# at-aaims/OmniFed

Hardware: AMD Instinct MI355X
Metric: GB/s device-resident QSGD encode+decode, Llama-400M grads, 1/2/4/8 GPUs (higher is better)
Workload: dtype f32; 1 GPU; llama400m QSGD encode+decode, bit_width 4 (16 levels, int8 wire), philox draws, client weighting fused (alpha = batch_samples = rank + 1), one client per GPU; tensors=183, elements_per_client=401122304, bit_width=4, parallelism=clients1

## Files before the change

omnifed_amd/csrc/omf_qsgd_bracket.hip:

```cpp
#include <algorithm>
#include <cstdlib>

#include "omf_bracket.h"
#include "omf_common.h"
#include "omf_plan.h"
#include "omf_qsgd_dec.h"
#include "omf_qsgd_dev.h"
#include "omf_qsgd_enc.h"

using namespace omf;
using namespace omf::plan_layout;

namespace {

constexpr int kSpecV = 4;
static_assert(kSpecBlk == (int64_t)kSpecV * kThreads * 4, "4096 elements per block");
constexpr int kSpecPerWaveWide = 32;
__host__ __device__ constexpr int spec_slot_words(int pw) { return pw == kSpecPerWave ? kSpecSlot : kWaves * pw; }
constexpr int64_t kSpecExact = 16384;

struct SpecArgs {
  EncArgs e;
  const int64_t* begins;
  const int64_t* sizes;
  const SpecBrItem* br_items;
  const SpecFoldItem* fold_items;
  SpecBracket* br;
  uint64_t* seg_part;
  uint32_t* fold_cnt;
  uint64_t* partials;
  uint32_t* heads;
  uint32_t* slots;
  float4* recs;
  uint32_t* flags;
  uint32_t* status;
  uint64_t* ngran;
  uint64_t wait_ticks;
  uint32_t dbg;
  float divisor;
  float zsig;
  float* xout;
  uint32_t epoch;
  uint32_t wide;
  double* br_part;
  uint64_t* brgran;
  uint32_t* br_cnt;
  int64_t nblocks;
  const void* aq;
  const float* anorm;
  float* aout;
  float alevels, ainv;
  int32_t awidth;
};

template <int AW, bool FULL>
__device__ __forceinline__ int4 acc_load(const void* q, int64_t e, int64_t end) {
  if (AW == 1) {
    const int8_t* q8 = static_cast<const int8_t*>(q);
    if (FULL || e + 4 <= end)
      return make_int4(__builtin_nontemporal_load(reinterpret_cast<const int32_t*>(q8 + e)), 0, 0, 0);
    uint32_t w = 0;
    for (int c = 0; c < 3; ++c)
      if (e + c < end) w |= (uint32_t)(uint8_t)q8[e + c] << (8 * c);
    return make_int4((int32_t)w, 0, 0, 0);
  }
  const int32_t* q32 = static_cast<const int32_t*>(q);
  if (FULL || e + 4 <= end) {
    const i32x4_t t = __builtin_nontemporal_load(reinterpret_cast<const i32x4_t*>(q32 + e));
    return make_int4(t[0], t[1], t[2], t[3]);
  }
  int4 r = make_int4(0, 0, 0, 0);
  if (e < end) r.x = q32[e];
  if (e + 1 < end) r.y = q32[e + 1];
  if (e + 2 < end) r.z = q32[e + 2];
  return r;
}

template <int AW>
__device__ __forceinline__ float4 acc_add4(float4 v, int4 raw, float norm, float alevels, float ainv) {
  int32_t qi[4];
  if (AW == 1) {
    qsgd_split_i8(raw.x, qi);
  } else {
    qi[0] = raw.x; qi[1] = raw.y; qi[2] = raw.z; qi[3] = raw.w;
  }
  float y[4];
#pragma unroll
  for (int c = 0; c < 4; ++c)
    y[c] = ainv != 0.0f ? qsgd_dec_elem<true>(norm, qi[c], alevels, ainv) : qsgd_dec_elem<false>(norm, qi[c], alevels, ainv);
  return make_float4(__fadd_rn(v.x, y[0]), __fadd_rn(v.y, y[1]), __fadd_rn(v.z, y[2]), __fadd_rn(v.w, y[3]));
}

__device__ __forceinline__ float4 br_value(const SpecArgs& a, float4 v, int64_t e, int64_t end, int32_t t) {
  if (!a.aq) return v;
  const float nrm = a.anorm[t];
  if (a.awidth == 32) return acc_add4<4>(v, acc_load<4, false>(a.aq, e, end), nrm, a.alevels, a.ainv);
  return acc_add4<1>(v, acc_load<1, false>(a.aq, e, end), nrm, a.alevels, a.ainv);
}

__device__ __forceinline__ uint32_t spec_hash(uint32_t a, uint32_t b) {
  uint32_t h = a * 0x9E3779B1u ^ (b + 0x7F4A7C15u) * 0x85EBCA77u;
  h ^= h >> 15; h *= 0x2C1B3C6Du; h ^= h >> 12; h *= 0x297A2D39u; h ^= h >> 15;
  return h;
}


__device__ __forceinline__ float4 scale_alpha(float4 v, float alpha) {
  if (alpha != 1.0f) {
    v.x = __fmul_rn(v.x, alpha); v.y = __fmul_rn(v.y, alpha);
    v.z = __fmul_rn(v.z, alpha); v.w = __fmul_rn(v.w, alpha);
  }
  return v;
}

__device__ __forceinline__ float4 spec_prologue(float4 v, float alpha, float divisor, uint32_t fmt) {
  v = scale_alpha(v, alpha);
  if (fmt && alpha != 1.0f) v = round_fmt4(v, fmt);
  if (divisor != 0.0f) {
    v.x = __fdiv_rn(v.x, divisor); v.y = __fdiv_rn(v.y, divisor);
    v.z = __fdiv_rn(v.z, divisor); v.w = __fdiv_rn(v.w, divisor);
  }
  return v;
}



template <int N>
__device__ __forceinline__ bool arrive_last(uint64_t* all, int32_t row, int64_t slot, const double (&v)[N],
                                            uint32_t* cnt, int32_t t, int parts) {
  uint64_t* mine = all + N * ((int64_t)row * parts + slot);
#pragma unroll
  for (int i = 0; i < N; ++i) st_agent(mine + i, (uint64_t)__double_as_longlong(v[i]));
  drain_vmem();
  const bool last = add_agent(&cnt[t], 1u) == (uint32_t)(parts - 1);
  if (last) __hip_atomic_store(&cnt[t], 0u, __ATOMIC_RELAXED, __HIP_MEMORY_SCOPE_AGENT);
  return last;
}
template <int N>
__device__ __forceinline__ bool arrive_last_block(uint64_t* all, int32_t row, int64_t slot, const double (&v)[N],
                                                  uint32_t* cnt, int32_t t, int parts, uint32_t& s_last) {
  if (threadIdx.x == 0) s_last = arrive_last(all, row, slot, v, cnt, t, parts) ? 1u : 0u;
  __syncthreads();
  return s_last != 0u;
}
__device__ __forceinline__ void combine_parts(const uint64_t* all, int32_t row, int parts, double (&S)[2]) {
  S[0] = S[1] = 0.0;
  for (int g = 0; g < parts; ++g) {
    const uint64_t* bp = all + 2 * ((int64_t)row * parts + g);
    S[0] += __longlong_as_double((long long)ld_agent(bp));
    S[1] += __longlong_as_double((long long)ld_agent(bp + 1));
  }
}

constexpr int kBrThreads = 1024;
constexpr int kBrWaves = kBrThreads / 64;

__device__ __forceinline__ double br_sum(double v, double* lds) {
  v = wave_sum_f64(v);
  if ((threadIdx.x & 63) == 0) lds[threadIdx.x >> 6] = v;
  __syncthreads();
  double s = 0.0;
#pragma unroll
  for (int w = 0; w < kBrWaves; ++w) s += lds[w];
  __syncthreads();
  return s;
}

template <int RUN, bool AQ, int NT = kBrThreads, int PASSES = 8>
__device__ __forceinline__ void bracket_sample(const SpecArgs& a, const float* __restrict__ x, int32_t t, int64_t tb,
                                               int64_t n, int64_t R, int part, int parts, double& s1, double& s2) {
  constexpr int LPR = RUN / 4, RPP = NT / LPR, PER_ROUND = RPP * PASSES;
  const int64_t base = n / R, rem = n % R;
  const int j = threadIdx.x & (LPR - 1);
  const float alpha = a.e.alpha;
  for (int64_t rb = (int64_t)part * PER_ROUND; rb < R; rb += (int64_t)parts * PER_ROUND) {
    float4 v[PASSES];
    bool live[PASSES];
    auto run_pos = [&](int i) {
      const int64_t r0 = rb + (int64_t)i * RPP + (threadIdx.x / LPR);
      const int64_t r = r0 < R ? r0 : 0;
      const int64_t lo = r * base + min(r, rem), len = base + (r < rem ? 1 : 0);
      return ((lo + (int64_t)(spec_hash((uint32_t)r, (uint32_t)t) % (uint32_t)(len - (RUN - 1)))) & ~(int64_t)3) + 4 * j;
    };
#pragma unroll
    for (int i = 0; i < PASSES; ++i) {
      live[i] = rb + (int64_t)i * RPP + (threadIdx.x / LPR) < R;
      v[i] = *reinterpret_cast<const float4*>(x + run_pos(i));
    }
    if (AQ) {
#pragma unroll
      for (int i = 0; i < PASSES; ++i) v[i] = br_value(a, v[i], tb + run_pos(i), tb + n, t);
    }
#pragma unroll
    for (int i = 0; i < PASSES; ++i) {
      float sr = live[i] ? sq4(spec_prologue(v[i], alpha, a.divisor, a.e.fmt), 0.0f) : 0.0f;
#pragma unroll
      for (int o = LPR / 2; o > 0; o >>= 1) sr += __shfl_xor(sr, o, LPR);
      if (live[i] && j == 0) {
        s1 += (double)sr;
        s2 += (double)sr * (double)sr;
      }
    }
  }
}

__device__ SpecBracket bracket_from_sums(const SpecArgs& a, bool exact, int64_t n, int64_t R, int run, double S1,
                                         double S2);

template <bool WIDE, bool AQ>
__device__ __forceinline__ void spec_bracket_body(const SpecArgs& a, const SpecBrItem* __restrict__ items,
                                                  double* red, uint32_t& s_last) {
  const int parts = WIDE ? kBrParts : 1;
  const int part = (int)(blockIdx.x % (unsigned)parts);
  const SpecBrItem bi = items[blockIdx.x / (unsigned)parts];
  const int32_t t = bi.tensor;
  const int64_t tb = bi.begin, n = bi.n;
  const float* __restrict__ x = a.e.x + tb;
  const float alpha = a.e.alpha;
  double s1 = 0.0, s2 = 0.0;
  const bool exact = n <= kSpecExact;
  const int64_t R = WIDE ? (int64_t)bi.Rw : (int64_t)bi.R;
  if (exact) {
    constexpr int PER = (int)(kSpecExact / (4 * kBrThreads));
    float4 v[PER];
    const int64_t nq = n & ~(int64_t)3;
#pragma unroll
    for (int i = 0; i < PER; ++i) {
      const int64_t e = 4 * ((int64_t)i * kBrThreads + threadIdx.x);
      v[i] = nq ? *reinterpret_cast<const float4*>(x + (e < nq ? e : 0)) : make_float4(0.f, 0.f, 0.f, 0.f);
    }
#pragma unroll
    for (int i = 0; i < PER; ++i) {
      const int64_t e = 4 * ((int64_t)i * kBrThreads + threadIdx.x);
      if (e >= nq) {
        v[i] = make_float4(0.f, 0.f, 0.f, 0.f);
        if (e < n) {
          v[i].x = x[e];
          if (e + 1 < n) v[i].y = x[e + 1];
          if (e + 2 < n) v[i].z = x[e + 2];
        }
      }
    }
    if (AQ) {
#pragma unroll
      for (int i = 0; i < PER; ++i) {
        const int64_t e = 4 * ((int64_t)i * kBrThreads + threadIdx.x);
        if (e < n) v[i] = br_value(a, v[i], tb + e, tb + n, t);
      }
    }
    float acc = 0.0f;
#pragma unroll
    for (int i = 0; i < PER; ++i) acc = sq4(spec_prologue(v[i], alpha, a.divisor, a.e.fmt), acc);
    s1 = acc;
  } else {
    bracket_sample<WIDE ? kSpecRunWide : kSpecRun, AQ>(a, x, t, tb, n, R, part, parts, s1, s2);
  }
  if (exact && part != 0) return;
  double S[2];
  S[0] = br_sum(s1, red);
  S[1] = br_sum(s2, red);
  if (!exact && parts > 1) {
    uint64_t* bp = reinterpret_cast<uint64_t*>(a.br_part);
    if (!arrive_last_block(bp, t, part, S, a.br_cnt, t, parts, s_last) || threadIdx.x != 0) return;
    combine_parts(bp, t, parts, S);
  }
  if (threadIdx.x != 0) return;
  a.br[t] = bracket_from_sums(a, exact, n, R, WIDE ? kSpecRunWide : kSpecRun, S[0], S[1]);
}

__device__ SpecBracket bracket_from_sums(const SpecArgs& a, bool exact, int64_t n, int64_t R, int run, double S1,
                                         double S2) {
  double ss, k;
  if (exact) {
    ss = S1;
    k = 0x1p-12;
  } else {
    const double Rd = (double)R, m = S1 / Rd;
    const double var = fmax(0.0, (S2 - Rd * m * m) / (Rd - 1.0));
    ss = S1 * ((double)n / ((double)run * Rd));
    k = (double)a.zsig * sqrt(var / Rd) / m + 0x1p-10;
  }
  const uint32_t fmt = a.e.fmt;
  const double kf = fmt == kFmtBF16 ? 0x1p-7 + 0x1p-14 : (fmt == kFmtF16 ? 0x1p-10 + 0x1p-20 : 0.0);
  const double mf = fmt == kFmtBF16 ? 0x1p-8 + 0x1p-16 : (fmt == kFmtF16 ? 0x1p-11 + 0x1p-22 : 0.0);
  k += kf;
  SpecBracket o{0.f, 0.f, 0.f, 0.f, 1u, {0u, 0u, 0u}};
  if (ss > 0.0 && ss < 1e300 && k < 0.5) {
    const float n_lo = nextafterf((float)sqrt(ss * (1.0 - k)), 0.0f);
    const float n_hi = nextafterf((float)sqrt(ss * (1.0 + k)), INFINITY);
    if (n_lo >= 0x1p-90f && n_hi < INFINITY) {
      const double L = (double)a.e.levels;
      o.n_lo = n_lo;
      o.n_hi = n_hi;
      o.c_lo = nextafterf((float)(L / (double)n_hi * (1.0 - 0x1p-20) * (1.0 - mf)), 0.0f);
      o.c_hi = nextafterf((float)(L / (double)n_lo * (1.0 + 0x1p-20) * (1.0 + mf)), INFINITY);
      o.mode = 0u;
    }
  }
  return o;
}

template <bool WIDE, bool AQ>
__global__ __launch_bounds__(kBrThreads) void qsgd_spec_bracket(SpecArgs a, const SpecBrItem* __restrict__ items) {
  __shared__ double red[kBrWaves];
  __shared__ uint32_t s_last;
  spec_bracket_body<WIDE, AQ>(a, items, red, s_last);
}
__global__ __launch_bounds__(kBrThreads) __attribute__((amdgpu_waves_per_eu(8))) void qsgd_spec_bracket_wide(
    SpecArgs a, const SpecBrItem* __restrict__ items) {
  __shared__ double red[kBrWaves];
  __shared__ uint32_t s_last;
  spec_bracket_body<true, false>(a, items, red, s_last);
}

__device__ __forceinline__ float raise_u(float u) {
  return __uint_as_float(max(__float_as_uint(u), 0x32800000u));
}
__device__ __forceinline__ void spec_quad(float4 x, float4 u, float c_lo, float c_hi, int32_t (&q)[4], uint64_t& und) {
  const float xs[4] = {x.x, x.y, x.z, x.w}, us[4] = {u.x, u.y, u.z, u.w};
#pragma unroll
  for (int c = 0; c < 4; ++c) {
    const float ax = fabsf(xs[c]);
    const float kl = ceilf(fmaf(ax, c_lo, -raise_u(us[c])));
    const float kh = ceilf(fmaf(ax, c_hi, -us[c]));
    und |= __builtin_amdgcn_fcmpf(kl, kh, 14 );
    q[c] = (int32_t)copysignf(kh, xs[c]);
  }
}

__device__ __forceinline__ void spec_quad_fmt(float4 x, float4 u, float c_lo, float c_hi, float dl, int32_t (&q)[4],
                                              uint64_t& und) {
  const float xs[4] = {x.x, x.y, x.z, x.w}, us[4] = {u.x, u.y, u.z, u.w};
#pragma unroll
  for (int c = 0; c < 4; ++c) {
    const float ax = fabsf(xs[c]);
    const float kl = ceilf(fmaf(ax, c_lo, -(raise_u(us[c]) + dl)));
    const float kh = ceilf(fmaf(ax, c_hi, dl - us[c]));
    und |= __builtin_amdgcn_fcmpf(kl, kh, 14 );
    q[c] = (int32_t)copysignf(kh, xs[c]);
  }
}


template <int WIDTH, bool FULL, bool DIV, uint32_t FMT, int AW = 0, int PW = kSpecPerWave, class GetBr>
__device__ __forceinline__ void spec_block(const SpecArgs& a, int64_t blk, int64_t b, int64_t end, int32_t t,
                                           int64_t tb, GetBr get_br, uint32_t* slot, uint64_t* part, float anorm,
                                           int tid) {
  const EncArgs& e = a.e;
  const int lane = tid & 63;
  const int wave = __builtin_amdgcn_readfirstlane(tid >> 6);
  float4 v[kSpecV];
  load_f4<kSpecV, FULL, true>(e.x, b, end, v, tid);
  int4 araw[AW ? kSpecV : 1];
  if (AW) {
#pragma unroll
    for (int k = 0; k < kSpecV; ++k)
      araw[k] = acc_load<AW ? AW : 1, FULL>(a.aq, b + 4 * ((int64_t)k * kThreads + tid), end);
  }
  float4 uu[4];
  philox_rows(e, b, tb, t, 0, uu, tid);
  const float alpha = e.alpha;
  float acc = 0.0f;
#pragma unroll
  for (int k = 0; k < kSpecV; ++k) {
    v[k] = mul4(v[k], alpha);
    if (FMT != kFmtF32 && alpha != 1.0f) v[k] = round_fmt4(v[k], FMT);
    if (AW) {
      v[k] = acc_add4<AW ? AW : 1>(v[k], araw[k], anorm, a.alevels, a.ainv);
      if (a.aout) {
        const int64_t el = b + 4 * ((int64_t)k * kThreads + tid);
        if (FULL || el + 4 <= end) {
          store_nt(a.aout + el, v[k]);
        } else if (el < end) {
          a.aout[el] = v[k].x;
          if (el + 1 < end) a.aout[el + 1] = v[k].y;
          if (el + 2 < end) a.aout[el + 2] = v[k].z;
        }
      }
    }
    if (DIV) {
      const float d = a.divisor;
      v[k].x = __fdiv_rn(v[k].x, d); v[k].y = __fdiv_rn(v[k].y, d);
      v[k].z = __fdiv_rn(v[k].z, d); v[k].w = __fdiv_rn(v[k].w, d);
      const int64_t el = b + 4 * ((int64_t)k * kThreads + tid);
      if (FULL || el + 4 <= end) {
        store_nt(a.xout + el, v[k]);
      } else if (el < end) {
        a.xout[el] = v[k].x;
        if (el + 1 < end) a.xout[el + 1] = v[k].y;
        if (el + 2 < end) a.xout[el + 2] = v[k].z;
      }
    }
    acc = sq4(v[k], acc);
  }
  const SpecBracket br = get_br();
  uint32_t cnt = 0;
  {
    uint32_t* list = slot + PW * wave;
#pragma unroll
    for (int k = 0; k < kSpecV; ++k) {
      const int64_t el = b + 4 * ((int64_t)k * kThreads + tid);
      const bool live = FULL || el < end;
      int32_t qq[4];
      uint64_t m = 0;
      if (FMT == kFmtF32) spec_quad(v[k], uu[k], br.c_lo, br.c_hi, qq, m);
      else spec_quad_fmt(v[k], uu[k], br.c_lo, br.c_hi, FMT == kFmtF16 ? 0x1p-25f * e.levels : 0.0f, qq, m);
      if (live) store_quad<WIDTH, FULL>(e, el, end, qq);
      if (!FULL) m &= __builtin_amdgcn_ballot_w64(live);
      if (m) {
        const bool und = (m >> lane) & 1ull;
        const uint32_t pos =
            cnt + __builtin_amdgcn_mbcnt_hi((uint32_t)(m >> 32), __builtin_amdgcn_mbcnt_lo((uint32_t)m, 0u));
        if (live && und && pos < (uint32_t)PW) {
          list[pos] = (uint32_t)(el >> 2);
          float4* rec = a.recs + 2 * ((blk * kWaves + wave) * PW + pos);
          rec[0] = v[k];
          rec[1] = uu[k];
        }
        cnt += (uint32_t)__popcll(m);
      }
    }
  }
  const double s = wave_sum_f64((double)acc);
  if (lane == 0) {
    *part = (uint64_t)__double_as_longlong(s);
    a.heads[blk * kWaves + wave] = ((uint32_t)t << 8) | min(cnt, (uint32_t)PW);
    if (cnt > (uint32_t)PW)
      __hip_atomic_fetch_or(&a.flags[t], 1u, __ATOMIC_RELAXED, __HIP_MEMORY_SCOPE_AGENT);
  }
}

template <int WIDTH, bool DIV, uint32_t FMT = kFmtF32, int AW = 0, int PW = kSpecPerWave, int WPB = kWaves>
__global__ __launch_bounds__(64 * WPB) void qsgd_spec_quant(SpecArgs a, const SpecBracket* __restrict__ brs,
                                                            const int64_t* __restrict__ begins,
                                                            const float* __restrict__ anorms) {
  static_assert(kWaves % WPB == 0, "a block's waves split evenly");
  constexpr int kPer = kWaves / WPB;
  const int64_t blk = blockIdx.x / kPer;
  const int tid = (int)(blockIdx.x % kPer) * 64 * WPB + (int)threadIdx.x;
  const Item it = a.e.items[blk >> 2];
  const SpecBracket br = brs[it.tensor];
  const int64_t tb = begins[it.tensor];
  const float anorm = AW ? anorms[it.tensor] : 0.0f;
  const int64_t b = it.begin + (blk & 3) * kSpecBlk;
  const int wave = tid >> 6;
  uint32_t* slot = a.slots + blk * spec_slot_words(PW);
  uint64_t* part = a.partials + blk * kWaves + wave;
  if (b >= it.end) {
    if ((tid & 63) == 0) {
      *part = 0ull;
      a.heads[blk * kWaves + wave] = (uint32_t)it.tensor << 8;
    }
    return;
  }
  const int64_t end = min(b + kSpecBlk, it.end);
  auto get_br = [&]() { return br; };
  if (end - b == kSpecBlk)
    spec_block<WIDTH, true, DIV, FMT, AW, PW>(a, blk, b, end, it.tensor, tb, get_br, slot, part, anorm, tid);
  else
    spec_block<WIDTH, false, DIV, FMT, AW, PW>(a, blk, b, end, it.tensor, tb, get_br, slot, part, anorm, tid);
}

#ifndef OMF_WFB_PASSES
#define OMF_WFB_PASSES 8
#endif
constexpr int kPassesW = OMF_WFB_PASSES;

template <int NT>
__device__ __forceinline__ double whole_sumsq(const SpecArgs& a, const float* __restrict__ x, int64_t n) {
  double s = 0.0;
  for (int64_t r0 = 0; r0 < n; r0 += 16 * NT) {
    float4 v[4];
#pragma unroll
      for (int i = 0; i < 4; ++i) {
        const int64_t e = r0 + 4 * ((int64_t)i * NT + threadIdx.x);
        v[i] = e + 4 <= n ? *reinterpret_cast<const float4*>(x + e) : make_float4(0.f, 0.f, 0.f, 0.f);
        if (e < n && e + 4 > n) {
          v[i].x = x[e];
          if (e + 1 < n) v[i].y = x[e + 1];
          if (e + 2 < n) v[i].z = x[e + 2];
        }
      }
    float acc = 0.0f;
#pragma unroll
    for (int i = 0; i < 4; ++i) acc = sq4(spec_prologue(v[i], a.e.alpha, a.divisor, a.e.fmt), acc);
    s += (double)acc;
  }
  return s;
}

template <int NT, int PARTS, int RUN, int PASSES>
__device__ __forceinline__ void spec_bracket_part(const SpecArgs& a, const SpecBrItem* __restrict__ items, int64_t wg) {
  static_assert(NT == 64 || NT == kThreads, "one wave, or block_sum_f64's workgroup");
  const int part = (int)(wg % PARTS);
  const SpecBrItem bi = items[wg / PARTS];
  const int32_t t = bi.tensor;
  const int64_t tb = bi.begin, n = bi.n, R = RUN == kSpecRunWide ? bi.Rw : bi.R;
  const float* __restrict__ x = a.e.x + tb;
  const bool exact = n <= kSpecExact;
  if (exact && part != 0) return;
  double s1 = 0.0, s2 = 0.0;
  if (exact) s1 = whole_sumsq<NT>(a, x, n);
  else bracket_sample<RUN, false, NT, PASSES>(a, x, t, tb, n, R, part, PARTS, s1, s2);
  double S[2];
  if constexpr (NT == 64) {
    S[0] = wave_sum_f64(s1);
    S[1] = wave_sum_f64(s2);
    if (threadIdx.x != 0) return;
  } else {
    __shared__ double red[kWaves];
    S[0] = block_sum_f64(s1, red);
    S[1] = block_sum_f64(s2, red);
  }
  if (!exact) {
    uint64_t* bp = reinterpret_cast<uint64_t*>(a.br_part);
    bool last;
    if constexpr (NT == 64) {
      last = arrive_last(bp, t, part, S, a.br_cnt, t, PARTS);
    } else {
      __shared__ uint32_t s_last;
      last = arrive_last_block(bp, t, part, S, a.br_cnt, t, PARTS, s_last);
    }
    if (!last) return;
    combine_parts(bp, t, PARTS, S);
  }
  if (threadIdx.x != 0) return;
  const SpecBracket o = bracket_from_sums(a, exact, n, R, RUN, S[0], S[1]);
  a.br[t] = o;
  const uint64_t ep = (uint64_t)a.epoch << 32;
  st_agent(&a.brgran[2 * t], ep | __float_as_uint(o.c_lo));
  st_agent(&a.brgran[2 * t + 1], ep | __float_as_uint(o.c_hi));
}

__device__ __forceinline__ SpecBracket fb_poll(const SpecArgs& a, int32_t t) {
  uint64_t g0 = ld_agent(&a.brgran[2 * t]), g1 = ld_agent(&a.brgran[2 * t + 1]);
  if ((uint32_t)(g0 >> 32) != a.epoch || (uint32_t)(g1 >> 32) != a.epoch) {
    const uint64_t t0 = wall_clock64(), min_polls = a.wait_ticks >> 10;
    uint64_t polls = 0;
    for (int k = 0;; k = min(k + 1, 6)) {
      if (k < 2) __builtin_amdgcn_s_sleep(2);
      else __builtin_amdgcn_s_sleep(8);
      g0 = ld_agent(&a.brgran[2 * t]);
      g1 = ld_agent(&a.brgran[2 * t + 1]);
      if ((uint32_t)(g0 >> 32) == a.epoch && (uint32_t)(g1 >> 32) == a.epoch) break;
      if (++polls > min_polls && wall_clock64() - t0 > a.wait_ticks) {
        __hip_atomic_fetch_or(&a.flags[t], 2u, __ATOMIC_RELAXED, __HIP_MEMORY_SCOPE_AGENT);
        g0 = g1 = 0;
        break;
      }
    }
  }
  return SpecBracket{__uint_as_float((uint32_t)g0), __uint_as_float((uint32_t)g1), 0.f, 0.f, 0u, {0u, 0u, 0u}};
}

template <int WIDTH, bool DIV, int PW>
__device__ __forceinline__ void fused_pass_block(const SpecArgs& a, int64_t blk, int tid,
                                                 const int64_t* __restrict__ begins) {
  const Item it = a.e.items[blk >> 2];
  const int32_t t = it.tensor;
  const int64_t tb = begins[t];
  const int64_t b = it.begin + (blk & 3) * kSpecBlk;
  const int wave = tid >> 6;
  uint32_t* slot = a.slots + blk * spec_slot_words(PW);
  uint64_t* part = a.partials + blk * kWaves + wave;
  if (b >= it.end) {
    if ((tid & 63) == 0) {
      *part = 0ull;
      a.heads[blk * kWaves + wave] = (uint32_t)t << 8;
    }
    return;
  }
  auto get_br = [&]() { return fb_poll(a, t); };
  const int64_t end = min(b + kSpecBlk, it.end);
  if (end - b == kSpecBlk)
    spec_block<WIDTH, true, DIV, kFmtF32, 0, PW>(a, blk, b, end, t, tb, get_br, slot, part, 0.0f, tid);
  else
    spec_block<WIDTH, false, DIV, kFmtF32, 0, PW>(a, blk, b, end, t, tb, get_br, slot, part, 0.0f, tid);
}

template <int WIDTH, bool DIV>
__global__ __launch_bounds__(kThreads) void qsgd_spec_quant_fb(SpecArgs a, const SpecBrItem* __restrict__ bitems,
                                                               int64_t nbrw, const int64_t* __restrict__ begins) {
  if ((int64_t)blockIdx.x < nbrw) {
    spec_bracket_part<kThreads, kFbParts, kSpecRun, 4>(a, bitems, blockIdx.x);
    return;
  }
  fused_pass_block<WIDTH, DIV, kSpecPerWave>(a, (int64_t)blockIdx.x - nbrw, (int)threadIdx.x, begins);
}

template <int WIDTH, bool DIV>
__global__ __launch_bounds__(64) void qsgd_spec_quant_wfb(SpecArgs a, const SpecBrItem* __restrict__ bitems,
                                                          int64_t nbrw, const int64_t* __restrict__ begins) {
  if ((int64_t)blockIdx.x < nbrw) {
    spec_bracket_part<64, kWfbParts, kSpecRunWide, kPassesW>(a, bitems, blockIdx.x);
    return;
  }
  const int64_t wgi = (int64_t)blockIdx.x - nbrw;
  fused_pass_block<WIDTH, DIV, kSpecPerWaveWide>(a, wgi / kWaves, (int)(wgi % kWaves) * 64 + (int)threadIdx.x, begins);
}

__device__ void spec_fold(const SpecArgs& a, const SpecFoldItem& fi) {
  __shared__ double red[kWaves];
  __shared__ uint32_t s_last;
  const int32_t t = fi.tensor;
  constexpr int U = kSpecSeg / kThreads;
  double v[U];
#pragma unroll
  for (int i = 0; i < U; ++i) {
    const int64_t j = fi.p_begin + threadIdx.x + (int64_t)i * kThreads;
    const double d = __longlong_as_double((long long)a.partials[j < fi.p_end ? j : fi.p_begin]);
    v[i] = j < fi.p_end ? d : 0.0;
  }
  double p = 0.0;
#pragma unroll
  for (int i = 0; i < U; ++i) p += v[i];
  double tot = block_sum_f64(p, red);
  if (fi.nsegs > 1) {
    const double seg[1] = {tot};
    if (!arrive_last_block(a.seg_part, 0, fi.sbase + fi.seg, seg, a.fold_cnt, t, fi.nsegs, s_last)) return;
    double q = 0.0;
    for (int j = threadIdx.x; j < fi.nsegs; j += kThreads)
      q += __longlong_as_double((long long)ld_agent(&a.seg_part[fi.sbase + j]));
    tot = block_sum_f64(q, red);
  }
  if (threadIdx.x != 0) return;
  const float norm = finish_norm(tot, a.e.fmt);
  a.e.norm_out[t] = norm;
  const SpecBracket br = a.br[t];
  const uint32_t fl = a.flags[t];
  const bool ok = br.mode == 0u && fl == 0u && norm >= br.n_lo && norm <= br.n_hi;
  a.status[t] = ok ? 0u : 1u;
  if (fl) a.flags[t] = 0u;
  st_agent(&a.ngran[t], ((uint64_t)((a.epoch << 1) | (ok ? 0u : 1u)) << 32) | __float_as_uint(norm));
}

__device__ __forceinline__ bool spec_norm_wait(const SpecArgs& a, int32_t t, float& norm, bool& bad) {
  uint64_t g = ld_agent(&a.ngran[t]);
  if ((uint32_t)(g >> 33) != a.epoch) {
    const uint64_t t0 = wall_clock64();
    const uint64_t min_polls = a.wait_ticks >> 10;
    uint64_t polls = 0;
    for (int k = 0;; k = min(k + 1, 6)) {
      if (k < 2) __builtin_amdgcn_s_sleep(4);
      else if (k < 4) __builtin_amdgcn_s_sleep(16);
      else __builtin_amdgcn_s_sleep(64);
      g = ld_agent(&a.ngran[t]);
      if ((uint32_t)(g >> 33) == a.epoch) break;
      if (++polls > min_polls && wall_clock64() - t0 > a.wait_ticks) {
        __hip_atomic_fetch_or(a.e.err, 4u, __ATOMIC_RELAXED, __HIP_MEMORY_SCOPE_AGENT);
        return false;
      }
    }
  }
  norm = __uint_as_float((uint32_t)g);
  bad = ((g >> 32) & 1u) != 0u;
  return true;
}

template <int WIDTH, int PW = kSpecPerWave, int FT = 1>
__global__ __launch_bounds__(kThreads) void qsgd_spec_finish(SpecArgs a, const SpecFoldItem* __restrict__ fold_items,
                                                             int32_t nfold, const Item* __restrict__ items,
                                                             const int64_t* __restrict__ begins,
                                                             const uint32_t* __restrict__ slots,
                                                             const float4* __restrict__ recs,
                                                             const uint32_t* __restrict__ heads) {
  if ((int32_t)blockIdx.x < nfold) {
    if (!(a.dbg & 16u)) spec_fold(a, fold_items[blockIdx.x]);
    return;
  }
  constexpr int BPW = kThreads / (kWaves * FT);
  __shared__ uint32_t s_rep[BPW];
  __shared__ float s_rep_norm[BPW];
  __shared__ uint32_t s_nrep;
  const EncArgs& e = a.e;
  const int64_t fb = (int64_t)blockIdx.x - nfold;
  if (threadIdx.x == 0) s_nrep = 0u;
  const int64_t ws = (fb * kThreads + threadIdx.x) / FT;
  const uint32_t sub = (uint32_t)(threadIdx.x % FT);
  const int64_t blk = ws / kWaves;
  const int w = (int)(ws % kWaves);
  bool rep = false;
  float rep_norm = 0.0f;
  if (blk < a.nblocks) {
    const uint32_t head = heads[ws];
    const uint32_t cnt = head & 0xffu;
    const int32_t t = (int32_t)(head >> 8);
    const bool leader = w == 0 && sub == 0;
    if ((cnt > 0u || leader) && !(a.dbg & 8u)) {
      constexpr int PRE = FT > 1 ? PW / FT : 0;
      uint32_t qv[PRE > 0 ? PRE : 1];
      float4 rx[PRE > 0 ? PRE : 1], ru[PRE > 0 ? PRE : 1];
      const uint32_t jl = cnt > 0u ? cnt - 1u : 0u;
#pragma unroll
      for (int k = 0; k < PRE; ++k) {
        const uint32_t j = min(sub + (uint32_t)(k * FT), jl);
        qv[k] = slots[blk * spec_slot_words(PW) + PW * w + j];
        rx[k] = recs[2 * (ws * PW + j)];
        ru[k] = recs[2 * (ws * PW + j) + 1];
      }
      const Item it = items[blk >> 2];
      float norm;
      bool bad;
      if (spec_norm_wait(a, t, norm, bad)) {
        const int64_t b = it.begin + (blk & 3) * kSpecBlk, end = min(b + kSpecBlk, it.end);
        const Divisor dv(norm, e.fmt);
#pragma unroll
        for (int k = 0; k < PRE; ++k) {
          if (sub + (uint32_t)(k * FT) >= cnt) break;
          int32_t qq[4];
          qsgd_quad<false>(rx[k], ru[k], dv, e.levels, false, qq);
          if (!(a.dbg & 4u)) store_quad<WIDTH>(e, 4 * (int64_t)qv[k], end, qq);
        }
        for (uint32_t j = sub + (uint32_t)(PRE * FT); j < cnt; j += FT) {
          const uint32_t q = slots[blk * spec_slot_words(PW) + PW * w + j];
          const float4* rec = recs + 2 * (ws * PW + j);
          int32_t qq[4];
          qsgd_quad<false>(rec[0], rec[1], dv, e.levels, false, qq);
          if (!(a.dbg & 4u)) store_quad<WIDTH>(e, 4 * (int64_t)q, end, qq);
        }
        rep = leader && bad;
        rep_norm = norm;
      }
    }
  }
  __syncthreads();
  if (rep) {
    const uint32_t i = atomicAdd(&s_nrep, 1u);
    s_rep[i] = (uint32_t)(blk - fb * BPW);
    s_rep_norm[i] = rep_norm;
  }
  if (!__syncthreads_or(rep)) return;
  const uint32_t nrep = s_nrep;
  EncArgs er = e;
  if (a.divisor != 0.0f) {
    er.x = a.xout;
    er.alpha = 1.0f;
  }
  for (uint32_t r = 0; r < nrep; ++r) {
    const int64_t rb = fb * BPW + s_rep[r];
    const Item it = items[rb >> 2];
    const int64_t b = it.begin + (rb & 3) * kSpecBlk;
    if (b < it.end)
      quant_sub<WIDTH, false, kSpecV>(er, b, min(b + kSpecBlk, it.end), begins[it.tensor], it.tensor, s_rep_norm[r]);
  }
}

}

static int ensure_wide(omf_plan* p, hipStream_t st) {
  if (p->d_spec_slots_w) return OMF_OK;
  const size_t nt = (size_t)p->nt, nb = (size_t)p->n_spec_blocks;
  Carve c;
  c.raw(p->d_spec_slots_w, (size_t)spec_slot_words(kSpecPerWaveWide) * nb);
  c.raw(p->d_spec_recs_w, 2 * (size_t)kWaves * kSpecPerWaveWide * nb);
  c.raw(p->d_spec_br_part, 2 * (size_t)kBrParts * nt);
  c.zero(p->d_spec_br_cnt, nt);
  return make_buffers(p, c, st);
}

static int ensure_fused_bracket(omf_plan* p, hipStream_t st) {
  if (p->d_spec_fb_part) return OMF_OK;
  const size_t nt = (size_t)p->nt;
  Carve c;
  c.raw(p->d_spec_fb_part, 2 * (size_t)std::max(kFbParts, kWfbParts) * nt);
  c.zero(p->d_spec_fb_cnt, nt);
  c.zero(p->d_spec_brgran, 2 * nt);
  return make_buffers(p, c, st);
}

int omf::bracket::launch(omf_plan* p, const EncCall& c, const Choice& ch) {
  using BracketKernel = void (*)(SpecArgs, const SpecBrItem*);
  using PassKernel = void (*)(SpecArgs, const SpecBracket*, const int64_t*, const float*);
  using FusedKernel = void (*)(SpecArgs, const SpecBrItem*, int64_t, const int64_t*);
  using FinishKernel = void (*)(SpecArgs, const SpecFoldItem*, int32_t, const Item*, const int64_t*, const uint32_t*,
                                const float4*, const uint32_t*);
  constexpr int PWW = kSpecPerWaveWide;
#ifndef OMF_FIX_FT
#define OMF_FIX_FT 4
#endif
  constexpr int FT = OMF_FIX_FT;
  static const BracketKernel k_bracket[2] = {qsgd_spec_bracket<false, false>, qsgd_spec_bracket<false, true>};
  static const FusedKernel k_fb[2] = {qsgd_spec_quant_fb<1, false>, qsgd_spec_quant_fb<1, true>};
  static const FusedKernel k_wfb[2][2] = {{qsgd_spec_quant_wfb<1, false>, qsgd_spec_quant_wfb<1, true>},
                                          {qsgd_spec_quant_wfb<4, false>, qsgd_spec_quant_wfb<4, true>}};
  static const PassKernel k_pass[2][2] = {{qsgd_spec_quant<1, false>, qsgd_spec_quant<1, true>},
                                          {qsgd_spec_quant<4, false>, qsgd_spec_quant<4, true>}};
  static const PassKernel k_pass_half[2] = {qsgd_spec_quant<1, false, kFmtBF16>, qsgd_spec_quant<1, false, kFmtF16>};
  static const PassKernel k_pass_last[2] = {qsgd_spec_quant<1, true, kFmtF32, 1>,
                                            qsgd_spec_quant<1, true, kFmtF32, 4>};
  static const PassKernel k_pass_wide[2][2][2] = {
      {{qsgd_spec_quant<1, false, kFmtF32, 0, PWW, 1>, qsgd_spec_quant<1, true, kFmtF32, 0, PWW, 1>},
       {qsgd_spec_quant<4, false, kFmtF32, 0, PWW, 1>, qsgd_spec_quant<4, true, kFmtF32, 0, PWW, 1>}},
      {{qsgd_spec_quant<1, false, kFmtF32, 0, PWW>, qsgd_spec_quant<1, true, kFmtF32, 0, PWW>},
       {qsgd_spec_quant<4, false, kFmtF32, 0, PWW>, qsgd_spec_quant<4, true, kFmtF32, 0, PWW>}}};
  static const FinishKernel k_finish[2][2] = {{qsgd_spec_finish<1>, qsgd_spec_finish<4>},
                                              {qsgd_spec_finish<1, PWW, FT>, qsgd_spec_finish<4, PWW, FT>}};
  static const size_t plds_w = [] { const char* v = omf::knob("OMF_SPEC_LDS_W"); return v ? (size_t)atoi(v) : (size_t)10240; }();
  static const size_t plds_n = [] { const char* v = omf::knob("OMF_SPEC_LDS"); return v ? (size_t)atoi(v) : (size_t)24576; }();
  static const bool wpb4 = [] { const char* v = omf::knob("OMF_SPEC_WPB"); return v && atoi(v) == 4; }();

  const hipStream_t st = c.st;
  const AccIn* acc = c.acc_in;
  const bool wide = ch.wide, div = c.divisor != 0.0f, w4 = c.width == 4;
  if (wide)
    if (int r = ensure_wide(p, st)) return r;
  if (ch.fused)
    if (int r = ensure_fused_bracket(p, st)) return r;
  SpecArgs sa;
  sa.e = enc_args(p, c);
  sa.e.items = p->d_flat;
  sa.e.tinfo = p->d_tinfo[1];
  sa.begins = p->d_begins;
  sa.sizes = p->d_sizes;
  sa.br_items = p->d_spec_br_items;
  sa.fold_items = p->d_spec_fold_items;
  sa.seg_part = p->d_spec_seg_part;
  sa.fold_cnt = p->d_spec_cnt;
  if (++p->spec_epoch >= 0x80000000u) p->spec_epoch = 1;
  sa.epoch = p->spec_epoch;
  sa.wide = wide ? 1u : 0u;
  sa.ngran = p->d_spec_ngran;
  sa.dbg = p->spec_skip;
  sa.zsig = wide ? p->spec_zsig_wide : p->spec_zsig;
  sa.divisor = c.divisor;
  sa.xout = c.xout;
  sa.wait_ticks = p->wait_ticks;
  sa.br = p->d_spec_br;
  sa.partials = p->d_spec_part;
  sa.br_part = ch.fused ? p->d_spec_fb_part : p->d_spec_br_part;
  sa.br_cnt = ch.fused ? p->d_spec_fb_cnt : p->d_spec_br_cnt;
  sa.brgran = p->d_spec_brgran;
  p->spec_last_pw = wide ? kSpecPerWaveWide : kSpecPerWave;
  sa.slots = wide ? p->d_spec_slots_w : p->d_spec_slots;
  sa.heads = p->d_spec_heads;
  sa.recs = wide ? p->d_spec_recs_w : p->d_spec_recs;
  sa.flags = p->d_spec_flags;
  sa.status = p->d_spec_status;
  sa.nblocks = p->n_spec_blocks;
  sa.aq = acc ? acc->q : nullptr;
  sa.anorm = acc ? acc->norm : nullptr;
  sa.aout = acc ? acc->acc_out : nullptr;
  sa.awidth = acc ? acc->width : 0;
  sa.alevels = acc ? (float)acc->levels : 0.0f;
  sa.ainv = acc && (acc->levels & (acc->levels - 1)) == 0 ? 1.0f / (float)acc->levels : 0.0f;

  const int64_t nb = p->n_spec_blocks, nt = p->nt;
  if (ch.bracket_launch)
    launch_kernel(wide ? qsgd_spec_bracket_wide : k_bracket[acc != nullptr], dim3((unsigned)(nt * (wide ? kBrParts : 1))),
           dim3(kBrThreads), 0, st, sa, sa.br_items);
  if (ch.fused) {
    const int64_t nbrw = (wide ? kWfbParts : kFbParts) * nt;
    if (wide) launch_kernel(k_wfb[w4][div], dim3((unsigned)(nbrw + nb * kWaves)), dim3(64), plds_w, st, sa, sa.br_items, nbrw, sa.begins);
    else launch_kernel(k_fb[div], dim3((unsigned)(nbrw + nb)), dim3(kThreads), div ? 0 : plds_n, st, sa, sa.br_items, nbrw, sa.begins);
  } else if (wide && !wpb4) {
    launch_kernel(k_pass_wide[0][w4][div], dim3((unsigned)(nb * kWaves)), dim3(64), plds_w, st, sa, sa.br, sa.begins, sa.anorm);
  } else {
    const PassKernel k = wide                 ? k_pass_wide[1][w4][div]
                         : c.fmt == kFmtBF16 ? k_pass_half[0]
                         : c.fmt == kFmtF16  ? k_pass_half[1]
                         : acc               ? k_pass_last[acc->width == 32]
                                             : k_pass[w4][div];
    launch_kernel(k, dim3((unsigned)nb), dim3(kThreads), 0, st, sa, sa.br, sa.begins, sa.anorm);
  }
  if (!(p->spec_skip & 2u)) {
    const int64_t per = kThreads / (kWaves * (wide ? FT : 1));
    const int32_t nfold = (int32_t)p->n_spec_fold;
    launch_kernel(k_finish[wide][w4], dim3((unsigned)(nfold + (nb + per - 1) / per)), dim3(kThreads), 0, st, sa, sa.fold_items,
           nfold, sa.e.items, sa.begins, sa.slots, sa.recs, sa.heads);
  }
  OMF_HIP(hipGetLastError());
  return OMF_OK;
}
```

Before: 6408 GB/s.

## Centralize norm polling per item in finish kernel and flatten sleep backoff

The finish kernel now has one lane per item poll the tensor norm flag and share the norm and status through shared memory, instead of every wave polling on its own. Slot and record prefetches are issued before the barrier so they overlap the wait. The fold path hoists the bracket and flag loads and issues the first segment load early, and the polling loop uses a fixed short sleep instead of escalating backoff. The goal is less redundant agent-scope polling and lower wake-up latency, at the cost of an extra block barrier and a poll loop that spins harder.

```diff
diff --git a/omnifed_amd/csrc/omf_qsgd_bracket.hip b/omnifed_amd/csrc/omf_qsgd_bracket.hip
--- a/omnifed_amd/csrc/omf_qsgd_bracket.hip
+++ b/omnifed_amd/csrc/omf_qsgd_bracket.hip
@@ -611,6 +611,8 @@
     const double d = __longlong_as_double((long long)a.partials[j < fi.p_end ? j : fi.p_begin]);
     v[i] = j < fi.p_end ? d : 0.0;
   }
+  const SpecBracket br = a.br[t];
+  const uint32_t fl = a.flags[t];
   double p = 0.0;
 #pragma unroll
   for (int i = 0; i < U; ++i) p += v[i];
@@ -618,32 +620,33 @@
   if (fi.nsegs > 1) {
     const double seg[1] = {tot};
     if (!arrive_last_block(a.seg_part, 0, fi.sbase + fi.seg, seg, a.fold_cnt, t, fi.nsegs, s_last)) return;
+    const int j0 = (int)threadIdx.x;
+    const uint64_t g0 = ld_agent(&a.seg_part[fi.sbase + (j0 < fi.nsegs ? j0 : 0)]);
     double q = 0.0;
-    for (int j = threadIdx.x; j < fi.nsegs; j += kThreads)
+    q += j0 < fi.nsegs ? __longlong_as_double((long long)g0) : 0.0;
+    for (int j = j0 + kThreads; j < fi.nsegs; j += kThreads)
       q += __longlong_as_double((long long)ld_agent(&a.seg_part[fi.sbase + j]));
     tot = block_sum_f64(q, red);
   }
   if (threadIdx.x != 0) return;
   const float norm = finish_norm(tot, a.e.fmt);
   a.e.norm_out[t] = norm;
-  const SpecBracket br = a.br[t];
-  const uint32_t fl = a.flags[t];
   const bool ok = br.mode == 0u && fl == 0u && norm >= br.n_lo && norm <= br.n_hi;
   a.status[t] = ok ? 0u : 1u;
   if (fl) a.flags[t] = 0u;
   st_agent(&a.ngran[t], ((uint64_t)((a.epoch << 1) | (ok ? 0u : 1u)) << 32) | __float_as_uint(norm));
 }
 
-__device__ __forceinline__ bool spec_norm_wait(const SpecArgs& a, int32_t t, float& norm, bool& bad) {
-  uint64_t g = ld_agent(&a.ngran[t]);
+#ifndef OMF_FIN_SLEEP
+#define OMF_FIN_SLEEP 8
+#endif
+__device__ __forceinline__ bool spec_norm_wait(const SpecArgs& a, int32_t t, uint64_t g, float& norm, bool& bad) {
   if ((uint32_t)(g >> 33) != a.epoch) {
     const uint64_t t0 = wall_clock64();
     const uint64_t min_polls = a.wait_ticks >> 10;
     uint64_t polls = 0;
-    for (int k = 0;; k = min(k + 1, 6)) {
-      if (k < 2) __builtin_amdgcn_s_sleep(4);
-      else if (k < 4) __builtin_amdgcn_s_sleep(16);
-      else __builtin_amdgcn_s_sleep(64);
+    for (;;) {
+      __builtin_amdgcn_s_sleep(OMF_FIN_SLEEP);
       g = ld_agent(&a.ngran[t]);
       if ((uint32_t)(g >> 33) == a.epoch) break;
       if (++polls > min_polls && wall_clock64() - t0 > a.wait_ticks) {
@@ -679,51 +682,69 @@
   const uint32_t sub = (uint32_t)(threadIdx.x % FT);
   const int64_t blk = ws / kWaves;
   const int w = (int)(ws % kWaves);
-  bool rep = false;
-  float rep_norm = 0.0f;
-  if (blk < a.nblocks) {
-    const uint32_t head = heads[ws];
-    const uint32_t cnt = head & 0xffu;
-    const int32_t t = (int32_t)(head >> 8);
-    const bool leader = w == 0 && sub == 0;
-    if ((cnt > 0u || leader) && !(a.dbg & 8u)) {
-      constexpr int PRE = FT > 1 ? PW / FT : 0;
-      uint32_t qv[PRE > 0 ? PRE : 1];
-      float4 rx[PRE > 0 ? PRE : 1], ru[PRE > 0 ? PRE : 1];
-      const uint32_t jl = cnt > 0u ? cnt - 1u : 0u;
-#pragma unroll
-      for (int k = 0; k < PRE; ++k) {
-        const uint32_t j = min(sub + (uint32_t)(k * FT), jl);
-        qv[k] = slots[blk * spec_slot_words(PW) + PW * w + j];
-        rx[k] = recs[2 * (ws * PW + j)];
-        ru[k] = recs[2 * (ws * PW + j) + 1];
-      }
-      const Item it = items[blk >> 2];
-      float norm;
-      bool bad;
-      if (spec_norm_wait(a, t, norm, bad)) {
-        const int64_t b = it.begin + (blk & 3) * kSpecBlk, end = min(b + kSpecBlk, it.end);
-        const Divisor dv(norm, e.fmt);
-#pragma unroll
-        for (int k = 0; k < PRE; ++k) {
-          if (sub + (uint32_t)(k * FT) >= cnt) break;
-          int32_t qq[4];
-          qsgd_quad<false>(rx[k], ru[k], dv, e.levels, false, qq);
-          if (!(a.dbg & 4u)) store_quad<WIDTH>(e, 4 * (int64_t)qv[k], end, qq);
-        }
-        for (uint32_t j = sub + (uint32_t)(PRE * FT); j < cnt; j += FT) {
-          const uint32_t q = slots[blk * spec_slot_words(PW) + PW * w + j];
-          const float4* rec = recs + 2 * (ws * PW + j);
-          int32_t qq[4];
-          qsgd_quad<false>(rec[0], rec[1], dv, e.levels, false, qq);
-          if (!(a.dbg & 4u)) store_quad<WIDTH>(e, 4 * (int64_t)q, end, qq);
-        }
-        rep = leader && bad;
-        rep_norm = norm;
-      }
-    }
+  constexpr int IPW = BPW / 4;
+  static_assert(BPW % 4 == 0 && IPW <= 64 && (IPW & (IPW - 1)) == 0, "whole items; their pollers are lanes of one wave");
+  __shared__ float s_inorm[IPW];
+  __shared__ uint32_t s_istat[IPW];
+  const bool fix = !(a.dbg & 8u);
+  const int64_t ii = fb * IPW + (threadIdx.x & (IPW - 1)), nitems = a.nblocks >> 2;
+  const int32_t pt = items[min(ii, nitems - 1)].tensor;
+  uint32_t head = heads[min(ws, a.nblocks * kWaves - 1)];
+  asm volatile("" : "+v"(head));
+  const uint32_t cnt = blk < a.nblocks && fix ? head & 0xffu : 0u;
+  const bool poller = threadIdx.x < IPW && ii < nitems && fix;
+  uint64_t g;
+  if (poller) g = ld_agent(&a.ngran[pt]);
+  constexpr int PRE = FT > 1 ? PW / FT : 1;
+  uint32_t qv[PRE];
+  float4 rx[PRE], ru[PRE];
+  Item it;
+  const bool listed = sub < cnt;
+  if (listed) {
+    const uint32_t jl = cnt - 1u;
+#pragma unroll
+    for (int k = 0; k < PRE; ++k) {
+      const uint32_t j = min(sub + (uint32_t)(k * FT), jl);
+      qv[k] = slots[blk * spec_slot_words(PW) + PW * w + j];
+      rx[k] = recs[2 * (ws * PW + j)];
+      ru[k] = recs[2 * (ws * PW + j) + 1];
+    }
+    it = items[blk >> 2];
+  }
+  if (threadIdx.x < IPW) {
+    float norm = 0.0f;
+    uint32_t stat = 0u;
+    if (poller) {
+      bool bad = false;
+      if (spec_norm_wait(a, pt, g, norm, bad)) stat = bad ? 3u : 1u;
+    }
+    s_inorm[threadIdx.x] = norm;
+    s_istat[threadIdx.x] = stat;
   }
   __syncthreads();
+  const int li = (int)(blk - fb * BPW) >> 2;
+  const uint32_t stat = s_istat[li];
+  const float norm = s_inorm[li];
+  if (listed && (stat & 1u)) {
+    const int64_t b = it.begin + (blk & 3) * kSpecBlk, end = min(b + kSpecBlk, it.end);
+    const Divisor dv(norm, e.fmt);
+#pragma unroll
+    for (int k = 0; k < PRE; ++k) {
+      if (sub + (uint32_t)(k * FT) >= cnt) break;
+      int32_t qq[4];
+      qsgd_quad<false>(rx[k], ru[k], dv, e.levels, false, qq);
+      if (!(a.dbg & 4u)) store_quad<WIDTH>(e, 4 * (int64_t)qv[k], end, qq);
+    }
+    for (uint32_t j = sub + (uint32_t)(PRE * FT); j < cnt; j += FT) {
+      const uint32_t q = slots[blk * spec_slot_words(PW) + PW * w + j];
+      const float4* rec = recs + 2 * (ws * PW + j);
+      int32_t qq[4];
+      qsgd_quad<false>(rec[0], rec[1], dv, e.levels, false, qq);
+      if (!(a.dbg & 4u)) store_quad<WIDTH>(e, 4 * (int64_t)q, end, qq);
+    }
+  }
+  const bool rep = w == 0 && sub == 0 && blk < a.nblocks && stat == 3u;
+  const float rep_norm = norm;
   if (rep) {
     const uint32_t i = atomicAdd(&s_nrep, 1u);
     s_rep[i] = (uint32_t)(blk - fb * BPW);
```

After: 6429 GB/s (median of 6 runs). About the same (+0.3%).
